# Atten4Vis/LW-DETR

Measured on AMD Instinct MI355X. Metric: images/sec, higher is better.
Workload: dtype fp16; 1 GPU; LW-DETR-small inference forward + PostProcess, 640x640, batch 32/GPU, fp16, random-init weights (synthetic COCO-shaped input); global_batch=32, per_gpu_batch=32, parallelism=dp1, collective=none, launch_chains=2

## Files before the change

lw-detr_amd/csrc/gemm.hip:

```cpp
#include "common.h"
#include <cstdlib>
#include <atomic>
#include <type_traits>

int lwdetr_gemm_pt_try(const lwdetr_gemm_desc& d, int dtype, hipStream_t st, bool& taken);

namespace {

constexpr int BK = 32;

template <typename T> __device__ __forceinline__ float act_apply(float x, int act) {
    if (act == ACT_GELU) return gelu_for<T>(x);
    if (act == ACT_SILU) return x * __builtin_amdgcn_rcpf(1.f + __expf(-x));
    if (act == ACT_RELU) return x > 0.f ? x : 0.f;
    return x;
}

__device__ __forceinline__ bool row_offset(const lwdetr_gemm_seg& sg, long m, long& off) {
    if (sg.mode == LWDETR_OUT_LINEAR) { off = m * sg.ldo; return true; }
    if (sg.mode == LWDETR_OUT_HEADS) {
        const int b = (int)(m / sg.p0), t = (int)(m - (long)b * sg.p0);
        off = ((long)b * sg.p2 * sg.p0 + t) * sg.p1;
        return true;
    }
// ... 750 lines not shown
    if constexpr (SPLITK) {
        constexpr int SLD = BN + 4, SLD_T = 64 + 4, SLAB = 64 * 68;
        float* stg = (float*)smem;
        int* flag = (int*)smem + SLAB + 16;
        static_assert((SLAB + 32) * 4 <= LDS_ELEMS * (int)sizeof(T), "stage + flag fit the ring area");
        {
            float* sp = col_orient ? stg + (wn * WN + l15) * SLD_T + wm * WM + g * 4 : stg + (wm * WM + l15) * SLD + wn * WN + g * 4;
            const int fs = col_orient ? 16 * SLD_T : 16, ts = col_orient ? 16 : 16 * SLD;
#pragma unroll
            for (int f = 0; f < FT; ++f)
#pragma unroll
                for (int t = 0; t < TT; ++t) *(f32x4*)(sp + f * fs + t * ts) = acc[f][t];
        }
        __syncthreads();
        float* ws = (float*)d.splitk_ws;
        const long ntiles = (long)gridDim.x / nsl;
        int* cnt = (int*)(ws + ntiles * nsl * SLAB);
        float* slab = ws + ((long)tile * nsl + slice) * SLAB;
        for (int i = tid; i < SLAB / 4; i += 256) ((f32x4*)slab)[i] = ((const f32x4*)stg)[i];
        asm volatile("s_waitcnt vmcnt(0)" ::: "memory");
        __syncthreads();
        if (tid == 0) {
            __builtin_amdgcn_fence(__ATOMIC_RELEASE, "agent");
            asm volatile("s_waitcnt vmcnt(0)" ::: "memory");
            *flag = __hip_atomic_fetch_add(cnt + tile, 1, __ATOMIC_RELAXED, __HIP_MEMORY_SCOPE_AGENT);
        }
        __syncthreads();
        if (*flag != nsl - 1) return;
        if (tid == 0) __builtin_amdgcn_fence(__ATOMIC_ACQUIRE, "agent");
        __syncthreads();
        const float* s0 = ws + (long)tile * nsl * SLAB;
        for (int i = tid; i < SLAB / 4; i += 256) {
            f32x4 a = ((const f32x4*)s0)[i];
            for (int s2 = 1; s2 < nsl; ++s2) { const f32x4 b = ((const f32x4*)(s0 + (long)s2 * SLAB))[i]; a[0] += b[0]; a[1] += b[1]; a[2] += b[2]; a[3] += b[3]; }
            ((f32x4*)stg)[i] = a;
        }
        if (tid == 0) __hip_atomic_store(cnt + tile, 0, __ATOMIC_RELAXED, __HIP_MEMORY_SCOPE_AGENT);
        __syncthreads();
        epilogue_finish<T, BN, 256>(d, sg, col_orient, stg, m0, n0);
    } else {
        gemm_epilogue<T, BM, BN>(d, sg, col_orient, acc, smem, m0, n0);
    }
}

template <typename T> struct Mma32;
template <> struct Mma32<f16> {
    static __device__ __forceinline__ f32x16 k16(f16x8 a, f16x8 b, f32x16 c) { return __builtin_amdgcn_mfma_f32_32x32x16_f16(a, b, c, 0, 0, 0); }
};
template <> struct Mma32<bf16> {
    static __device__ __forceinline__ f32x16 k16(bf16x8 a, bf16x8 b, f32x16 c) { return __builtin_amdgcn_mfma_f32_32x32x16_bf16(a, b, c, 0, 0, 0); }
};

#ifdef LWDETR_CONV_TIMING
__device__ unsigned long long g_conv_timing[4][12];
extern "C" int lwdetr_debug_conv_timing(unsigned long long* out) {
    return hipMemcpyFromSymbol(out, HIP_SYMBOL(g_conv_timing), sizeof(g_conv_timing)) == hipSuccess ? 0 : -1;
}
#define CONV_NOW() __builtin_amdgcn_s_memrealtime()
#endif
#ifndef LWDETR_CONV_ABL
#define LWDETR_CONV_ABL 0
#endif
template <typename V8>
__device__ __forceinline__ void lds_read16(V8& dst, unsigned lds_addr) { asm volatile("ds_read_b128 %0, %1" : "=v"(dst) : "v"(lds_addr)); }
__device__ __forceinline__ void divmod_magic(unsigned n, unsigned dvs, unsigned magic, unsigned& q, unsigned& r) {
    q = __umulhi(n, magic); r = n - q * dvs;
    if (r >= dvs) { ++q; r -= dvs; }
}

template <typename T, int CIN, int BN, int NST>
__global__ __launch_bounds__(256) void conv3x3_patch_kernel(const lwdetr_gemm_desc d, int np_patch, unsigned magic_hw, unsigned magic_w) {
    constexpr int BM = 128, KB = 32, EPC = 8;
    constexpr int SPR = CIN / EPC + 1, RS = SPR * EPC;
    constexpr int NCH = CIN / KB;
    constexpr int B_MY = BN / 16 / 4;
    constexpr int WN = BN / 2, TM = 2, TN = WN / 32, NRD = TM + TN;
    typedef typename Vec<T>::v8 V8;
    static_assert(sizeof(T) == 2 && BN % 64 == 0 && CIN % KB == 0 && (NCH == 4 || NCH == 6), "16-bit, whole pieces, 4 or 6 stages per tap");
    extern __shared__ __attribute__((aligned(16))) unsigned char conv_smem[];
    T* patch = (T*)conv_smem;
    T* ring = patch + (long)np_patch * 512;
    const unsigned lds_patch = (unsigned)(uintptr_t)(__attribute__((address_space(3))) void*)conv_smem;
    const unsigned lds_ring = lds_patch + (unsigned)np_patch * 1024u;

    const int nwg = gridDim.x;
    int wg;
    {
        const int bid = blockIdx.x, q = nwg >> 3, r = nwg & 7, xcd = bid & 7;
        wg = (xcd < r ? xcd * (q + 1) : r * (q + 1) + (xcd - r) * q) + (bid >> 3);
    }
    const int m0 = wg * BM;
    const int tid = threadIdx.x, lane = tid & 63, wave = tid >> 6;
    const int l31 = lane & 31, h = lane >> 5;
    const int wm = wave >> 1, wn = wave & 1;
    const int Wimg = d.conv_wout, Himg = d.conv_hout, PR = BM + 2 * Wimg + 2;
    const T* __restrict__ A = (const T*)d.A + d.a_col0;
    const T* __restrict__ W = (const T*)d.W;
    const T* zero = (const T*)g_zero16;
#ifdef LWDETR_CONV_TIMING
    const unsigned long long ct0 = CONV_NOW(); unsigned long long ct_lgkm = 0, ct_vm = 0, ct_bar = 0;
#endif

    const int prow = lane >> 2, pslot = lane & 3;
    const T* w_src[B_MY];
#pragma unroll
    for (int k = 0; k < B_MY; ++k) {
        const int n = 16 * (wave + 4 * k) + prow;
        w_src[k] = n < d.N ? W + (long)n * d.K + (pslot ^ ((prow >> 2) & 3)) * EPC : nullptr;
    }
    const int nk = 9 * NCH;
    auto stage = [&](int kt, int slot) {
        T* Bs = ring + slot * (BN * KB);
#pragma unroll
        for (int k = 0; k < B_MY; ++k) {
            if (LWDETR_CONV_ABL & 8) continue;
            gdma16((kt < nk && w_src[k]) ? w_src[k] + kt * KB : zero, Bs + (wave + 4 * k) * 64 * EPC);
        }
    };
#pragma unroll
    for (int s = 0; s < NST; ++s) stage(s, s);
    {
        constexpr unsigned MAGIC_SPR = 0x100000000ull / SPR;
        constexpr int DR = 256 / SPR, DS = 256 - DR * SPR;
        const int lda = (int)d.lda, gm0 = m0 - Wimg - 1;
        unsigned pr, ps;
        divmod_magic((unsigned)(wave * 64 + lane), SPR, MAGIC_SPR, pr, ps);
        int goff = (gm0 + (int)pr) * lda + (int)ps * EPC;
        for (int p = wave; p < np_patch; p += 4) {
            const int gm = gm0 + (int)pr;
            const bool ok = ps < SPR - 1 && (int)pr < PR && gm >= 0 && gm < d.M;
            if (!(LWDETR_CONV_ABL & 2)) gdma16(ok ? A + goff : zero, patch + p * 512);
            pr += DR; ps += DS; goff += DR * lda + DS * EPC;
            if (ps >= SPR) { ps -= SPR; ++pr; goff += lda - SPR * EPC; }
        }
    }
#ifdef LWDETR_CONV_TIMING
    const unsigned long long ct1 = CONV_NOW();
#endif
    unsigned vbits[TM], need[TM];
    {
        const unsigned hw = (unsigned)(Himg * Wimg);
#pragma unroll
        for (int i = 0; i < TM; ++i) {
            unsigned qq, r, y, x;
            divmod_magic((unsigned)(m0 + wm * 64 + i * 32 + l31), hw, magic_hw, qq, r);
            divmod_magic(r, (unsigned)Wimg, magic_w, y, x);
            const bool top = y == 0, bot = (int)y == Himg - 1, lef = x == 0, rig = (int)x == Wimg - 1;
            const unsigned row_ok[3] = {top ? 0u : 7u, 7u, bot ? 0u : 7u};
            const unsigned col_ok = (lef ? 0u : 0x49u) | 0x92u | (rig ? 0u : 0x124u);
            vbits[i] = (row_ok[0] | row_ok[1] << 3 | row_ok[2] << 6) & col_ok;
            const unsigned at = __builtin_amdgcn_ballot_w64(top) != 0, ab = __builtin_amdgcn_ballot_w64(bot) != 0;
            const unsigned al = __builtin_amdgcn_ballot_w64(lef) != 0, ar = __builtin_amdgcn_ballot_w64(rig) != 0;
            need[i] = (at ? 7u : 0u) | (ab ? 7u << 6 : 0u) | (al ? 0x49u : 0u) | (ar ? 0x124u : 0u);
        }
    }
    unsigned a_addr[TM], w_addr[TN][2];
#pragma unroll
    for (int i = 0; i < TM; ++i) a_addr[i] = lds_patch + (unsigned)(((wm * 64 + i * 32 + l31) * RS + h * EPC) * (int)sizeof(T));
#pragma unroll
    for (int j = 0; j < TN; ++j)
#pragma unroll
        for (int kc = 0; kc < 2; ++kc)
            w_addr[j][kc] = lds_ring + (unsigned)(((wn * WN + j * 32 + l31) * KB + ((2 * kc + h) ^ ((l31 >> 2) & 3)) * EPC) * (int)sizeof(T));

    f32x16 acc[TN][TM];
#pragma unroll
    for (int j = 0; j < TN; ++j)
#pragma unroll
        for (int i = 0; i < TM; ++i)
#pragma unroll
            for (int e = 0; e < 16; ++e) acc[j][i][e] = 0.f;

#ifdef LWDETR_CONV_TIMING
    const unsigned long long ct2 = CONV_NOW();
#endif
    wait_vmcnt<0>();
    __builtin_amdgcn_s_barrier();
#ifdef LWDETR_CONV_TIMING
    const unsigned long long ct3 = CONV_NOW();
#endif
    auto load = [&](auto c_tag, auto kc_tag, const unsigned (&a_tap)[TM], unsigned soff, V8 (&xf)[TM], V8 (&wf)[TN]) {
// ... 31 lines not shown
            for (int j = 0; j < TN; ++j) asm volatile("" :: "v"(wf[j]));
#pragma unroll
            for (int i = 0; i < TM; ++i) asm volatile("" :: "v"(xf[i]));
            return;
        }
#pragma unroll
        for (int j = 0; j < TN; ++j)
#pragma unroll
            for (int i = 0; i < TM; ++i) acc[j][i] = Mma32<T>::k16(wf[j], xf[i], acc[j][i]);
    };
    auto tap_rows = [&](int tap, unsigned (&a_tap)[TM]) {
        const unsigned toff = (unsigned)((Wimg + 1 + (tap / 3 - 1) * Wimg + (tap % 3 - 1)) * RS * (int)sizeof(T));
#pragma unroll
        for (int i = 0; i < TM; ++i) a_tap[i] = a_addr[i] + toff;
    };
    constexpr unsigned SLOT_B = BN * KB * sizeof(T);
    V8 xa[TM], wa[TN], xb[TM], wb[TN];
    unsigned a_cur[TM], a_nxt[TM];
    tap_rows(0, a_cur);
    load(std::integral_constant<int, 0>{}, std::integral_constant<int, 0>{}, a_cur, 0u, xa, wa);
    int kt = 0;
    unsigned soff = 0;
#pragma unroll 1
    for (int tap = 0; tap < 9; ++tap) {
        tap_rows(tap + 1, a_nxt);
        unsigned nd[TM], keep[TM];
#pragma unroll
        for (int i = 0; i < TM; ++i) { nd[i] = (need[i] >> tap) & 1; keep[i] = (vbits[i] >> tap) & 1 ? 0xffffffffu : 0u; }
        auto one_stage = [&](auto c_tag) {
            constexpr int C = decltype(c_tag)::value;
            load(c_tag, std::integral_constant<int, 1>{}, a_cur, soff, xb, wb);
            landed(std::integral_constant<int, NRD>{}, xa, wa);
            mma(nd, keep, xa, wa);
#ifdef LWDETR_CONV_TIMING
            const unsigned long long cta = CONV_NOW();
#endif
            landed(std::integral_constant<int, 0>{}, xb, wb);
#ifdef LWDETR_CONV_TIMING
            const unsigned long long ctb = CONV_NOW();
#endif
            wait_vmcnt<(NST - 2) * B_MY>();
#ifdef LWDETR_CONV_TIMING
            const unsigned long long ctc = CONV_NOW();
#endif
            __builtin_amdgcn_s_barrier();
#ifdef LWDETR_CONV_TIMING
            ct_lgkm += ctb - cta; ct_vm += ctc - ctb; ct_bar += CONV_NOW() - ctc;
#endif
            {
                T* Bs = (T*)((unsigned char*)ring + soff);
#pragma unroll
                for (int k = 0; k < B_MY; ++k) {
                    if (LWDETR_CONV_ABL & 8) continue;
                    gdma16((kt + NST < nk && w_src[k]) ? w_src[k] + (kt + NST) * KB : zero, Bs + (wave + 4 * k) * 64 * EPC);
                }
            }
            soff = soff + SLOT_B == NST * SLOT_B ? 0u : soff + SLOT_B;
            ++kt;
            if constexpr (C + 1 < NCH) load(std::integral_constant<int, C + 1>{}, std::integral_constant<int, 0>{}, a_cur, soff, xa, wa);
            else if (tap < 8) load(std::integral_constant<int, 0>{}, std::integral_constant<int, 0>{}, a_nxt, soff, xa, wa);
            mma(nd, keep, xb, wb);
        };
        one_stage(std::integral_constant<int, 0>{});
        one_stage(std::integral_constant<int, 1>{});
        one_stage(std::integral_constant<int, 2>{});
        one_stage(std::integral_constant<int, 3>{});
        if constexpr (NCH > 4) { one_stage(std::integral_constant<int, 4>{}); one_stage(std::integral_constant<int, 5>{}); }
#pragma unroll
        for (int i = 0; i < TM; ++i) a_cur[i] = a_nxt[i];
    }
#ifdef LWDETR_CONV_TIMING
    const unsigned long long ct4 = CONV_NOW();
#endif
    wait_vmcnt<0>();
    __syncthreads();
    float* stg = (float*)conv_smem;
    constexpr int SLD = BN + 4;
    if (LWDETR_CONV_ABL & 4) {
        float keepalive = 0.f;
#pragma unroll
        for (int j = 0; j < TN; ++j)
#pragma unroll
            for (int i = 0; i < TM; ++i)
#pragma unroll
                for (int e = 0; e < 16; ++e) keepalive += acc[j][i][e];
        if (keepalive == 123.456f) stg[0] = 1.f;
        return;
    }
#pragma unroll 1
    for (int pass = 0; pass < 2; ++pass) {
        if (wm == pass) {
#pragma unroll
            for (int i = 0; i < TM; ++i)
#pragma unroll
                for (int j = 0; j < TN; ++j)
#pragma unroll
                    for (int q = 0; q < 4; ++q) {
                        const f32x4 v = {acc[j][i][4 * q], acc[j][i][4 * q + 1], acc[j][i][4 * q + 2], acc[j][i][4 * q + 3]};
                        *(f32x4*)(stg + (i * 32 + l31) * SLD + wn * WN + j * 32 + q * 8 + h * 4) = v;
                    }
        }
        __syncthreads();
        epilogue_finish<T, BN, 256>(d, d.seg[0], false, stg, m0 + pass * 64, 0);
        __syncthreads();
    }
#ifdef LWDETR_CONV_TIMING
    if (wg == LWDETR_CONV_TIMING && lane == 0) {
        unsigned long long* o = g_conv_timing[wave];
        const unsigned long long ct5 = CONV_NOW();
        o[0] = ct1 - ct0; o[1] = ct2 - ct1; o[2] = ct3 - ct2; o[3] = ct4 - ct3; o[4] = ct5 - ct4; o[5] = ct_lgkm; o[6] = ct_vm; o[7] = ct_bar; o[8] = ct5 - ct0;
    }
#endif
}




#ifndef LWDETR_BIG_VARIANT
#define LWDETR_BIG_VARIANT 0
#endif
#ifdef LWDETR_BIG_TIMING
__device__ unsigned long long g_big_timing[8][8];
extern "C" int lwdetr_debug_big_timing(unsigned long long* out) {
    return hipMemcpyFromSymbol(out, HIP_SYMBOL(g_big_timing), sizeof(g_big_timing)) == hipSuccess ? 0 : 1;
}
#define BIG_NOW() __builtin_amdgcn_s_memrealtime()
#endif
template <typename T, int BN, int KB, int NST, int AMODE, int BM, int NW, bool LN = false>
__device__ __forceinline__ void gemm_big_body(const lwdetr_gemm_desc& d) {
    static_assert(sizeof(T) == 2, "16-bit types only");
    static_assert((NW == 8 && BM == 256) || (NW == 4 && BM == 128), "8 waves x 256 rows or 4 waves x 128 rows");
    constexpr int EPC = 8;
    constexpr int WGN = BN == 256 ? 4 : 2, WGM = NW / WGN;
    constexpr int WM = BM / WGM, WN = BN / WGN, TM = WM / 32, TN = WN / 32;
    static_assert(WN % 32 == 0 && WM % 64 == 0 && (BN / (64 / (KB / 8))) % NW == 0 && (BM / (64 / (KB / 8))) % NW == 0, "tile / stage combination not supported");
    constexpr int SLOTS = KB / EPC, RP = 64 / SLOTS, KC = KB / 16;
    constexpr int A_MY = BM / RP / NW, B_MY = BN / RP / NW, PER_STAGE = A_MY + B_MY;
    constexpr int STAGE = (BM + BN) * KB;
    typedef typename Vec<T>::v8 V8;
    extern __shared__ __attribute__((aligned(16))) char big_smem[];
    T* smem = (T*)big_smem;

    const int tiles_n = (d.N + BN - 1) / BN;
    int wg;
    {
        const int nwg = gridDim.x, bid = blockIdx.x, q = nwg >> 3, r = nwg & 7, xcd = bid & 7;
        wg = (xcd < r ? xcd * (q + 1) : r * (q + 1) + (xcd - r) * q) + (bid >> 3);
    }
    const int tm_ = wg / tiles_n, tn_ = wg - tm_ * tiles_n;
    const long m0 = (long)tm_ * BM;
    const int n0 = tn_ * BN;
    const int tid = threadIdx.x, lane = tid & 63, wave = tid >> 6;
    const int m = lane & 31, h = lane >> 5;
    const int wm = wave / WGN, wn = wave % WGN;
    const T* __restrict__ A = (const T*)d.A;
    const T* __restrict__ W = (const T*)d.W;
    const T* zero = (const T*)g_zero16;
// ... 240 lines not shown
}

int g_big_mode = -1;
template <int AMODE>
bool big_2wg_pays(const lwdetr_gemm_desc& d, int bn) {
    (void)d; (void)bn;
    return false;
}
template <typename T, int AMODE>
int try_launch_big(const lwdetr_gemm_desc& d, hipStream_t st, bool& taken) {
    taken = false;
    if constexpr (sizeof(T) != 2 || AMODE == LWDETR_A_PATCH16) return LWDETR_OK;
    else {
        const int mode = g_big_mode >= 0 ? g_big_mode : (int)lwdetr_knob(KNOB_GEMM_BIG, 1);
        if (!mode || d.A2 || d.K % 64 != 0 || d.N < 128) return LWDETR_OK;
        if (AMODE == LWDETR_A_CONV3x3 && (d.conv_cin % 64 != 0 || d.a_col0 % 8 != 0 || d.conv_hout > 1024 || d.conv_wout > 1024 ||
                                          d.M / ((long)d.conv_hout * d.conv_wout) >= 2048)) return LWDETR_OK;
        int bn = d.N % 256 == 0 || d.N > 512 ? 256 : (d.N <= 192 ? 192 : 128);
        bn = (int)lwdetr_knob(KNOB_GEMM_BIG_BN, bn);
        for (int s = 0; s < d.nseg; ++s)
            if (d.seg[s].n_begin % bn != 0) bn = 128;
        for (int s = 0; s < d.nseg; ++s) if (d.seg[s].n_begin % bn != 0) return LWDETR_OK;
        const long tiles = ((d.M + 255) / 256) * ((d.N + bn - 1) / bn);
        if (mode == 1 && !(d.K >= 384 && d.N >= 192 && (d.M >= 16384 || (d.K >= 960 && tiles >= 96)))) return LWDETR_OK;
        const int variant = mode >= 10 ? mode : 0;
        const int wg2_mode = (int)lwdetr_knob(KNOB_GEMM_BIG_2WG, 1);
        const bool wg2 = variant == 128 || (variant == 0 && (wg2_mode == 2 || (wg2_mode == 1 && big_2wg_pays<AMODE>(d, bn))));
        int rc;
        bool ln = false;
        for (int s_ = 0; s_ < d.nseg; ++s_) ln = ln || d.seg[s_].ln_stats != nullptr;
        if (ln) {
#ifdef LWDETR_EXPERIMENTS
            if constexpr (AMODE == LWDETR_A_PLAIN) {
                if (bn == 256) { rc = launch_big<T, 256, 64, 2, LWDETR_A_PLAIN, 256, 8, true>(d, st); taken = rc != LWDETR_ERR_UNSUPPORTED; return taken ? rc : LWDETR_OK; }
            }
#endif
            return LWDETR_OK;
        }
#ifdef LWDETR_EXPERIMENTS
        if (wg2 && bn == 256) rc = launch_big<T, 256, 32, 3, AMODE, 128, 4>(d, st);
        else if (wg2 && bn == 192) rc = launch_big<T, 192, 32, 3, AMODE, 128, 4>(d, st);
        else
#else
        (void)wg2;
#endif
        if (bn == 256) rc = variant == 32 ? launch_big<T, 256, 32, 4, AMODE>(d, st) : launch_big<T, 256, 64, 2, AMODE>(d, st);
        else if (bn == 192) rc = launch_big<T, 192, 64, 2, AMODE>(d, st);
        else rc = variant == 32 ? launch_big<T, 128, 32, 4, AMODE>(d, st) : launch_big<T, 128, 64, 3, AMODE>(d, st);
        taken = rc != LWDETR_ERR_UNSUPPORTED;
        return taken ? rc : LWDETR_OK;
    }
}

template <typename T, int CIN, int NST>
int launch_conv_patch(const lwdetr_gemm_desc& d, hipStream_t st) {
    constexpr int SPR = CIN / 8 + 1;
    const int pr = 128 + 2 * d.conv_wout + 2;
    const int np = (pr * SPR + 63) / 64;
    size_t lds = (size_t)np * 1024 + (size_t)NST * CIN * 32 * sizeof(T);
    const size_t stg = (size_t)64 * (CIN + 4) * sizeof(float);
    if (lds < stg) lds = stg;
    if (lds > 160 * 1024) return LWDETR_ERR_UNSUPPORTED;
    static signed char state[16] = {};
    int dev = 0;
    if (hipGetDevice(&dev) != hipSuccess || dev < 0 || dev >= 16) return LWDETR_ERR_UNSUPPORTED;
    if (state[dev] == 0)
        state[dev] = hipFuncSetAttribute((const void*)conv3x3_patch_kernel<T, CIN, CIN, NST>, hipFuncAttributeMaxDynamicSharedMemorySize, 160 * 1024) == hipSuccess ? 1 : -1;
    if (state[dev] < 0) { (void)hipGetLastError(); return LWDETR_ERR_UNSUPPORTED; }
    const long nwg = (d.M + 127) / 128;
    const unsigned hw = (unsigned)(d.conv_hout * d.conv_wout);
    hipLaunchKernelGGL((conv3x3_patch_kernel<T, CIN, CIN, NST>), dim3((unsigned)nwg), dim3(256), lds, st, d, np,
                       (unsigned)(0x100000000ull / hw), (unsigned)(0x100000000ull / (unsigned)d.conv_wout));
    return lwdetr_gemm_path_done(CIN == 128 ? GP_CONV_PATCH_128 : GP_CONV_PATCH_192, lwdetr_check_launch());
}

template <typename T>
int try_launch_conv_patch(const lwdetr_gemm_desc& d, hipStream_t st, bool& taken) {
    taken = false;
    if constexpr (sizeof(T) != 2) return LWDETR_OK;
    else {
        const int mode = (int)lwdetr_knob(KNOB_CONV_PATCH, 1);
        if (mode == 0) return LWDETR_OK;
        if (mode == 1 && d.N != 128) return LWDETR_OK;
        if (mode == 1 && d.M < 100 * 128) return LWDETR_OK;
        const lwdetr_gemm_seg& g = d.seg[0];
        const long hw = (long)d.conv_hout * d.conv_wout;
        if (d.conv_stride != 1 || d.a_tok.winmajor || d.a_tok.Hp != d.conv_hout || d.a_tok.Wp != d.conv_wout || d.nseg != 1 ||
            g.mode != LWDETR_OUT_LINEAR || d.N != d.conv_cin || d.K != 9 * d.conv_cin || (d.N != 128 && d.N != 192) ||
            d.lda % 8 != 0 || d.a_col0 % 8 != 0 || ((size_t)d.A & 15) != 0 || ((size_t)d.W & 15) != 0 || hw <= 1 || d.M % hw != 0 ||
            d.conv_wout < 2 || (long)(d.M + 256) * d.lda >= (1L << 30))
            return LWDETR_OK;
        const int rc = d.N == 128 ? launch_conv_patch<T, 128, 3>(d, st) : launch_conv_patch<T, 192, 3>(d, st);
        taken = rc != LWDETR_ERR_UNSUPPORTED;
        return taken ? rc : LWDETR_OK;
    }
}

template <typename T, int AMODE>
int launch(const lwdetr_gemm_desc& d, hipStream_t st) {
    bool bn64 = d.N <= 64 || sizeof(T) == 4;
    for (int s = 0; s < d.nseg; ++s)
        if ((d.seg[s].n_begin % 128) != 0) bn64 = true;
    const int BNsel = bn64 ? 64 : 128;
    for (int s = 0; s < d.nseg; ++s)
        if (d.seg[s].n_begin % BNsel != 0) return LWDETR_ERR_UNSUPPORTED;
    long tiles_m = (d.M + 127) / 128, tiles_n = (d.N + BNsel - 1) / BNsel;
    bool small = AMODE != LWDETR_A_CONV3x3 || tiles_m * tiles_n < 384;
    if (lwdetr_knob_is_set(KNOB_GEMM_TILE)) {
        const int tsel = (int)lwdetr_knob(KNOB_GEMM_TILE, 0);
        if (tsel == 1) small = true;
        if (tsel == 2) { small = false; bn64 = true; tiles_n = (d.N + 63) / 64; }
        if (tsel == 3 && !bn64) small = false;
    }
    if (small) { tiles_m = (d.M + 63) / 64; tiles_n = (d.N + 63) / 64; }
    const long nwg = tiles_m * tiles_n;
    if (nwg <= 0 || nwg > 0x7fffffffL) return LWDETR_ERR_BAD_ARG;
    const int kid = AMODE == LWDETR_A_PLAIN ? KID_GEMM : (AMODE == LWDETR_A_CONV3x3 ? KID_GEMM_CONV : KID_GEMM_PATCH);
    ProfScope ps(kid, 2.0 * d.M * d.N * d.K, ((double)d.M * d.K + (double)d.N * d.K + (double)d.M * d.N) * sizeof(T), st);
    if constexpr (AMODE == LWDETR_A_CONV3x3) {
        bool taken = false;
        const int rc = try_launch_conv_patch<T>(d, st, taken);
        if (taken) return rc;
    }
    if constexpr (AMODE == LWDETR_A_PLAIN && sizeof(T) == 2) {
        bool taken = false;
        const int rc = lwdetr_gemm_pt_try(d, std::is_same<T, f16>::value ? DT_F16 : DT_BF16, st, taken);
        if (taken) return rc;
    }
    {
        bool taken = false;
        const int rc = try_launch_big<T, AMODE>(d, st, taken);
        if (taken) return rc;
        for (int s_ = 0; s_ < d.nseg; ++s_)
            if (d.seg[s_].ln_stats) return LWDETR_ERR_UNSUPPORTED;
    }
    if constexpr (sizeof(T) == 2) {
        const int mode = (int)lwdetr_knob(KNOB_GEMM_DMA, 3);
        if (mode && !d.A2) {
            const bool kb64 = lwdetr_knob(KNOB_GEMM_KB, 32) == 64 && d.K % 64 == 0 && (AMODE != LWDETR_A_CONV3x3 || d.conv_cin % 64 == 0);
            int path;
            if (small && kb64) { hipLaunchKernelGGL((gemm_dma_kernel<T, 64, 64, AMODE, 3, 64>), dim3((unsigned)nwg), dim3(256), 0, st, d); path = GP_RING_64x64_D3_KB64; }
            else if (small) {
                const int nst = (int)lwdetr_knob(KNOB_GEMM_NST, 3);
                if (nst == 2) { hipLaunchKernelGGL((gemm_dma_kernel<T, 64, 64, AMODE, 2>), dim3((unsigned)nwg), dim3(256), 0, st, d); path = GP_RING_64x64_D2; }
#ifdef LWDETR_EXPERIMENTS
// ... 101 lines not shown
```

lw-detr_amd/csrc/topk.hip:

```cpp
#include "common.h"

namespace {

constexpr int TK_THREADS = 1024;
constexpr int TK_MAXK = 1024;
constexpr int TK_IDX_BITS = 20;
constexpr unsigned TK_IDX_MASK = (1u << TK_IDX_BITS) - 1;

__device__ __forceinline__ unsigned fkey(float f) {
    const unsigned u = __float_as_uint(f);
    return (u & 0x80000000u) ? ~u : (u | 0x80000000u);
}
__device__ __forceinline__ float fkey_inv(unsigned k) {
    return __uint_as_float((k & 0x80000000u) ? (k ^ 0x80000000u) : ~k);
}

__device__ __forceinline__ unsigned long long tk_comp(unsigned key, int i) {
    return ((unsigned long long)key << TK_IDX_BITS) | (unsigned long long)(TK_IDX_MASK - (unsigned)i);
}

struct TopkShared {
    unsigned hist[2048];
    unsigned long long sel[TK_MAXK];
    unsigned rank[TK_MAXK];
    unsigned bstar, above, cnt, nsel;
};

template <typename T, bool CACHE>
__device__ void topk_block(const T* __restrict__ x, int N, int K, TopkShared& sh, unsigned* __restrict__ keys) {
    const int tid = threadIdx.x;
    unsigned long long prefix = 0;
    unsigned rem = (unsigned)K;
    unsigned long long thr = 0;
    int top = 32 + TK_IDX_BITS;
    bool first = true;
    while (true) {
        const int bits = top > 30 ? 11 : 10;
        const int shift = top - bits;
        const unsigned nb = 1u << bits;
        for (int i = tid; i < 2048; i += TK_THREADS) sh.hist[i] = 0;
        __syncthreads();
        if (first) {
            int i = tid;
            for (; i + 3 * TK_THREADS < N; i += 4 * TK_THREADS) {
                unsigned k4[4];
#pragma unroll
                for (int u = 0; u < 4; ++u) k4[u] = fkey(to_f32<T>(x[i + u * TK_THREADS]));
#pragma unroll
                for (int u = 0; u < 4; ++u) {
                    if (CACHE) keys[i + u * TK_THREADS] = k4[u];
                    atomicAdd(&sh.hist[k4[u] >> 21], 1u);
                }
            }
            for (; i < N; i += TK_THREADS) {
                const unsigned k = fkey(to_f32<T>(x[i]));
                if (CACHE) keys[i] = k;
                atomicAdd(&sh.hist[k >> 21], 1u);
            }
        } else {
            for (int i = tid; i < N; i += TK_THREADS) {
                const unsigned long long c = tk_comp(CACHE ? keys[i] : fkey(to_f32<T>(x[i])), i);
                if ((c >> top) == prefix) atomicAdd(&sh.hist[(unsigned)(c >> shift) & (nb - 1)], 1u);
            }
        }
        first = false;
        __syncthreads();
        if (tid < 64) {
            const int per = (int)nb >> 6;
            unsigned own = 0;
            for (int j = 0; j < per; ++j) own += sh.hist[tid * per + ((j + tid) & (per - 1))];
            unsigned s = own;
#pragma unroll
            for (int o = 1; o < 64; o <<= 1) {
                const unsigned t = __shfl_down(s, o);
                if (tid + o < 64) s += t;
            }
            const unsigned excl = s - own;
            if (excl < rem && rem <= s) {
                unsigned acc = excl;
                for (int j = per - 1; j >= 0; --j) {
                    const unsigned c = sh.hist[tid * per + j];
                    if (acc + c >= rem) { sh.bstar = (unsigned)(tid * per + j); sh.above = acc; sh.cnt = c; break; }
                    acc += c;
                }
            }
        }
        __syncthreads();
        const unsigned bstar = sh.bstar, above = sh.above, cnt = sh.cnt;
        rem -= above;
        prefix = (prefix << bits) | bstar;
        top = shift;
        if (cnt == rem || top == 0) { thr = prefix << top; break; }
    }
    if (tid == 0) sh.nsel = 0;
    for (int i = tid; i < TK_MAXK; i += TK_THREADS) sh.rank[i] = 0;
    __syncthreads();
    for (int i = tid; i < N; i += TK_THREADS) {
        const unsigned long long c = tk_comp(CACHE ? keys[i] : fkey(to_f32<T>(x[i])), i);
        if (c >= thr) {
            const unsigned p = atomicAdd(&sh.nsel, 1u);
            if (p < (unsigned)K) sh.sel[p] = c;
        }
    }
    __syncthreads();
    const int parts = TK_THREADS / K > 0 ? TK_THREADS / K : 1;
    const int e = tid % K, p = tid / K;
    if (p < parts) {
        const unsigned long long mine = sh.sel[e];
        const int j0 = (int)((long)K * p / parts), j1 = (int)((long)K * (p + 1) / parts);
        unsigned r = 0;
        for (int j = j0; j < j1; ++j) r += sh.sel[j] > mine ? 1u : 0u;
        atomicAdd(&sh.rank[e], r);
    }
    __syncthreads();
}

template <typename T, bool CACHE>
__global__ __launch_bounds__(TK_THREADS) void topk_kernel(const T* __restrict__ x, int N, int K, int64_t* __restrict__ idx_out,
                                                          float* __restrict__ val_out) {
    __shared__ TopkShared sh;
    extern __shared__ unsigned tk_keys[];
    const int b = blockIdx.x;
    topk_block<T, CACHE>(x + (long)b * N, N, K, sh, tk_keys);
    const int tid = threadIdx.x;
    if (tid < K) {
        const unsigned long long c = sh.sel[tid];
        const unsigned r = sh.rank[tid];
        idx_out[(long)b * K + r] = (int64_t)(TK_IDX_MASK - (unsigned)(c & TK_IDX_MASK));
        if (val_out) val_out[(long)b * K + r] = fkey_inv((unsigned)(c >> TK_IDX_BITS));
    }
}

template <typename T, bool CACHE>
__global__ __launch_bounds__(TK_THREADS) void postprocess_kernel(const T* __restrict__ logits, const T* __restrict__ boxes,
                                                                 const float* __restrict__ sizes, int nq, int ncls, int K,
                                                                 float* __restrict__ scores, int64_t* __restrict__ labels,
                                                                 float* __restrict__ out_boxes, float* __restrict__ packed) {
    __shared__ TopkShared sh;
    extern __shared__ unsigned tk_keys[];
    const int b = blockIdx.x;
    const int N = nq * ncls;
    topk_block<T, CACHE>(logits + (long)b * N, N, K, sh, tk_keys);
    const int tid = threadIdx.x;
    if (tid < K) {
        const unsigned long long c = sh.sel[tid];
        const long o = (long)b * K + sh.rank[tid];
        const int i = (int)(TK_IDX_MASK - (unsigned)(c & TK_IDX_MASK));
        const int q = i / ncls;
        const float v = fkey_inv((unsigned)(c >> TK_IDX_BITS));
        const float score = to_f32<T>(from_f32<T>(1.f / (1.f + expf(-v))));
        const T* bx = boxes + ((long)b * nq + q) * 4;
        const float cx = to_f32<T>(bx[0]), cy = to_f32<T>(bx[1]);
        const float w = fmaxf(to_f32<T>(bx[2]), 0.f), h = fmaxf(to_f32<T>(bx[3]), 0.f);
        const float ih = sizes[b * 2], iw = sizes[b * 2 + 1];
        const float x0 = to_f32<T>(from_f32<T>(cx - 0.5f * w)) * iw, y0 = to_f32<T>(from_f32<T>(cy - 0.5f * h)) * ih;
        const float x1 = to_f32<T>(from_f32<T>(cx + 0.5f * w)) * iw, y1 = to_f32<T>(from_f32<T>(cy + 0.5f * h)) * ih;
        if (packed) {
            float* pr = packed + o * 6;
            pr[0] = score; pr[1] = (float)(i - q * ncls); pr[2] = x0; pr[3] = y0; pr[4] = x1; pr[5] = y1;
        } else {
            scores[o] = score;
            labels[o] = (int64_t)(i - q * ncls);
            out_boxes[o * 4 + 0] = x0; out_boxes[o * 4 + 1] = y0; out_boxes[o * 4 + 2] = x1; out_boxes[o * 4 + 3] = y1;
        }
    }
}

template <typename T>
__global__ __launch_bounds__(256) void rowmax_kernel(const T* __restrict__ x, long ld, long rows, int ncols, float* __restrict__ out) {
    constexpr int EPC = 4;
    typedef T VC __attribute__((ext_vector_type(EPC)));
    const int lane16 = threadIdx.x & 15;
    const long row = (long)blockIdx.x * 16 + (threadIdx.x >> 4);
    float m = -INFINITY;
    if (row < rows) {
        const T* xr = x + row * ld;
        const int full = ncols / EPC;
        for (int c = lane16; c < full; c += 16) {
            const VC t = *(const VC*)(xr + c * EPC);
#pragma unroll
            for (int e = 0; e < EPC; ++e) m = fmaxf(m, to_f32<T>(t[e]));
        }
        for (int c = full * EPC + lane16; c < ncols; c += 16) m = fmaxf(m, to_f32<T>(xr[c]));
    }
#pragma unroll
    for (int o = 8; o >= 1; o >>= 1) m = fmaxf(m, __shfl_xor(m, o));
    if (row < rows && lane16 == 0) out[row] = m;
}

}

constexpr size_t TK_CACHE_BYTES = 160 * 1024 - sizeof(TopkShared) - 256;
static bool tk_allow_lds(const void* fn) {
    static const void* done[16]; static int ndone = 0;
    for (int i = 0; i < ndone; ++i) if (done[i] == fn) return true;
    if (hipFuncSetAttribute(fn, hipFuncAttributeMaxDynamicSharedMemorySize, (int)TK_CACHE_BYTES) != hipSuccess) return false;
    if (ndone < 16) done[ndone++] = fn;
    return true;
}

#define LWDETR_DISPATCH_T(dtype, CALL)                 \
    switch (dtype) {                                   \
// ... 69 lines not shown
```

Baseline: 14100 images/sec.

## Add 8-wave 256-row conv3x3 patch kernel variant for large 128-channel convs

Templates the patch-based 3x3 conv kernel on wave count, adding an 8-wave variant with a 256-row M tile that loads the input patch and weight stages with more threads and does a single-pass epilogue. The wide variant (with 4 weight stages) is picked for 128-channel convs when the number of 128-row tiles exceeds the CU count. The aim is to amortise the halo patch load and weight streaming over more output rows and cut the tail wave. It raises LDS use per block, which may lower occupancy.

```diff
diff --git a/lw-detr_amd/csrc/gemm.hip b/lw-detr_amd/csrc/gemm.hip
--- a/lw-detr_amd/csrc/gemm.hip
+++ b/lw-detr_amd/csrc/gemm.hip
@@ -826,7 +826,7 @@
 };
 
 #ifdef LWDETR_CONV_TIMING
-__device__ unsigned long long g_conv_timing[4][12];
+__device__ unsigned long long g_conv_timing[8][12];
 extern "C" int lwdetr_debug_conv_timing(unsigned long long* out) {
     return hipMemcpyFromSymbol(out, HIP_SYMBOL(g_conv_timing), sizeof(g_conv_timing)) == hipSuccess ? 0 : -1;
 }
@@ -834,6 +834,9 @@
 #endif
 #ifndef LWDETR_CONV_ABL
 #define LWDETR_CONV_ABL 0
+#endif
+#ifndef LWDETR_CONV8_NST
+#define LWDETR_CONV8_NST 4
 #endif
 template <typename V8>
 __device__ __forceinline__ void lds_read16(V8& dst, unsigned lds_addr) { asm volatile("ds_read_b128 %0, %1" : "=v"(dst) : "v"(lds_addr)); }
@@ -842,15 +845,16 @@
     if (r >= dvs) { ++q; r -= dvs; }
 }
 
-template <typename T, int CIN, int BN, int NST>
-__global__ __launch_bounds__(256) void conv3x3_patch_kernel(const lwdetr_gemm_desc d, int np_patch, unsigned magic_hw, unsigned magic_w) {
-    constexpr int BM = 128, KB = 32, EPC = 8;
+template <typename T, int CIN, int BN, int NST, int NW>
+__global__ __launch_bounds__(NW * 64) void conv3x3_patch_kernel(const lwdetr_gemm_desc d, int np_patch, unsigned magic_hw, unsigned magic_w) {
+    constexpr int BM = NW * 32, KB = 32, EPC = 8;
     constexpr int SPR = CIN / EPC + 1, RS = SPR * EPC;
     constexpr int NCH = CIN / KB;
-    constexpr int B_MY = BN / 16 / 4;
+    constexpr int B_MY = BN / 16 / NW;
     constexpr int WN = BN / 2, TM = 2, TN = WN / 32, NRD = TM + TN;
     typedef typename Vec<T>::v8 V8;
-    static_assert(sizeof(T) == 2 && BN % 64 == 0 && CIN % KB == 0 && (NCH == 4 || NCH == 6), "16-bit, whole pieces, 4 or 6 stages per tap");
+    static_assert(sizeof(T) == 2 && BN % 64 == 0 && (BN / 16) % NW == 0 && CIN % KB == 0 && (NCH == 4 || NCH == 6) && (NW == 4 || NW == 8),
+                  "16-bit, whole pieces per wave, 4 or 6 stages per tap, 4 or 8 waves");
     extern __shared__ __attribute__((aligned(16))) unsigned char conv_smem[];
     T* patch = (T*)conv_smem;
     T* ring = patch + (long)np_patch * 512;
@@ -879,7 +883,7 @@
     const T* w_src[B_MY];
 #pragma unroll
     for (int k = 0; k < B_MY; ++k) {
-        const int n = 16 * (wave + 4 * k) + prow;
+        const int n = 16 * (wave + NW * k) + prow;
         w_src[k] = n < d.N ? W + (long)n * d.K + (pslot ^ ((prow >> 2) & 3)) * EPC : nullptr;
     }
     const int nk = 9 * NCH;
@@ -888,19 +892,19 @@
 #pragma unroll
         for (int k = 0; k < B_MY; ++k) {
             if (LWDETR_CONV_ABL & 8) continue;
-            gdma16((kt < nk && w_src[k]) ? w_src[k] + kt * KB : zero, Bs + (wave + 4 * k) * 64 * EPC);
+            gdma16((kt < nk && w_src[k]) ? w_src[k] + kt * KB : zero, Bs + (wave + NW * k) * 64 * EPC);
         }
     };
 #pragma unroll
     for (int s = 0; s < NST; ++s) stage(s, s);
     {
         constexpr unsigned MAGIC_SPR = 0x100000000ull / SPR;
-        constexpr int DR = 256 / SPR, DS = 256 - DR * SPR;
+        constexpr int DR = NW * 64 / SPR, DS = NW * 64 - DR * SPR;
         const int lda = (int)d.lda, gm0 = m0 - Wimg - 1;
         unsigned pr, ps;
         divmod_magic((unsigned)(wave * 64 + lane), SPR, MAGIC_SPR, pr, ps);
         int goff = (gm0 + (int)pr) * lda + (int)ps * EPC;
-        for (int p = wave; p < np_patch; p += 4) {
+        for (int p = wave; p < np_patch; p += NW) {
             const int gm = gm0 + (int)pr;
             const bool ok = ps < SPR - 1 && (int)pr < PR && gm >= 0 && gm < d.M;
             if (!(LWDETR_CONV_ABL & 2)) gdma16(ok ? A + goff : zero, patch + p * 512);
@@ -1038,7 +1042,7 @@
 #pragma unroll
                 for (int k = 0; k < B_MY; ++k) {
                     if (LWDETR_CONV_ABL & 8) continue;
-                    gdma16((kt + NST < nk && w_src[k]) ? w_src[k] + (kt + NST) * KB : zero, Bs + (wave + 4 * k) * 64 * EPC);
+                    gdma16((kt + NST < nk && w_src[k]) ? w_src[k] + (kt + NST) * KB : zero, Bs + (wave + NW * k) * 64 * EPC);
                 }
             }
             soff = soff + SLOT_B == NST * SLOT_B ? 0u : soff + SLOT_B;
@@ -1061,7 +1065,7 @@
     wait_vmcnt<0>();
     __syncthreads();
     float* stg = (float*)conv_smem;
-    constexpr int SLD = BN + 4;
+    constexpr int SLD = BN + 4, EPR = NW == 8 ? BM : 64;
     if (LWDETR_CONV_ABL & 4) {
         float keepalive = 0.f;
 #pragma unroll
@@ -1074,8 +1078,9 @@
         return;
     }
 #pragma unroll 1
-    for (int pass = 0; pass < 2; ++pass) {
-        if (wm == pass) {
+    for (int pass = 0; pass < BM / EPR; ++pass) {
+        if (wm * 64 / EPR == pass) {
+            const int r0 = wm * 64 - pass * EPR;
 #pragma unroll
             for (int i = 0; i < TM; ++i)
 #pragma unroll
@@ -1083,12 +1088,13 @@
 #pragma unroll
                     for (int q = 0; q < 4; ++q) {
                         const f32x4 v = {acc[j][i][4 * q], acc[j][i][4 * q + 1], acc[j][i][4 * q + 2], acc[j][i][4 * q + 3]};
-                        *(f32x4*)(stg + (i * 32 + l31) * SLD + wn * WN + j * 32 + q * 8 + h * 4) = v;
+                        *(f32x4*)(stg + (r0 + i * 32 + l31) * SLD + wn * WN + j * 32 + q * 8 + h * 4) = v;
                     }
         }
         __syncthreads();
-        epilogue_finish<T, BN, 256>(d, d.seg[0], false, stg, m0 + pass * 64, 0);
-        __syncthreads();
+#pragma unroll
+        for (int s = 0; s < EPR / 64; ++s) epilogue_finish<T, BN, NW * 64>(d, d.seg[0], false, stg + s * 64 * SLD, m0 + pass * EPR + s * 64, 0);
+        if (pass + 1 < BM / EPR) __syncthreads();
     }
 #ifdef LWDETR_CONV_TIMING
     if (wg == LWDETR_CONV_TIMING && lane == 0) {
@@ -1435,24 +1441,24 @@
     }
 }
 
-template <typename T, int CIN, int NST>
+template <typename T, int CIN, int NST, int NW>
 int launch_conv_patch(const lwdetr_gemm_desc& d, hipStream_t st) {
-    constexpr int SPR = CIN / 8 + 1;
-    const int pr = 128 + 2 * d.conv_wout + 2;
+    constexpr int SPR = CIN / 8 + 1, BM = NW * 32;
+    const int pr = BM + 2 * d.conv_wout + 2;
     const int np = (pr * SPR + 63) / 64;
     size_t lds = (size_t)np * 1024 + (size_t)NST * CIN * 32 * sizeof(T);
-    const size_t stg = (size_t)64 * (CIN + 4) * sizeof(float);
+    const size_t stg = (size_t)(NW == 8 ? BM : 64) * (CIN + 4) * sizeof(float);
     if (lds < stg) lds = stg;
     if (lds > 160 * 1024) return LWDETR_ERR_UNSUPPORTED;
     static signed char state[16] = {};
     int dev = 0;
     if (hipGetDevice(&dev) != hipSuccess || dev < 0 || dev >= 16) return LWDETR_ERR_UNSUPPORTED;
     if (state[dev] == 0)
-        state[dev] = hipFuncSetAttribute((const void*)conv3x3_patch_kernel<T, CIN, CIN, NST>, hipFuncAttributeMaxDynamicSharedMemorySize, 160 * 1024) == hipSuccess ? 1 : -1;
+        state[dev] = hipFuncSetAttribute((const void*)conv3x3_patch_kernel<T, CIN, CIN, NST, NW>, hipFuncAttributeMaxDynamicSharedMemorySize, 160 * 1024) == hipSuccess ? 1 : -1;
     if (state[dev] < 0) { (void)hipGetLastError(); return LWDETR_ERR_UNSUPPORTED; }
-    const long nwg = (d.M + 127) / 128;
+    const long nwg = (d.M + BM - 1) / BM;
     const unsigned hw = (unsigned)(d.conv_hout * d.conv_wout);
-    hipLaunchKernelGGL((conv3x3_patch_kernel<T, CIN, CIN, NST>), dim3((unsigned)nwg), dim3(256), lds, st, d, np,
+    hipLaunchKernelGGL((conv3x3_patch_kernel<T, CIN, CIN, NST, NW>), dim3((unsigned)nwg), dim3(NW * 64), lds, st, d, np,
                        (unsigned)(0x100000000ull / hw), (unsigned)(0x100000000ull / (unsigned)d.conv_wout));
     return lwdetr_gemm_path_done(CIN == 128 ? GP_CONV_PATCH_128 : GP_CONV_PATCH_192, lwdetr_check_launch());
 }
@@ -1471,9 +1477,20 @@
         if (d.conv_stride != 1 || d.a_tok.winmajor || d.a_tok.Hp != d.conv_hout || d.a_tok.Wp != d.conv_wout || d.nseg != 1 ||
             g.mode != LWDETR_OUT_LINEAR || d.N != d.conv_cin || d.K != 9 * d.conv_cin || (d.N != 128 && d.N != 192) ||
             d.lda % 8 != 0 || d.a_col0 % 8 != 0 || ((size_t)d.A & 15) != 0 || ((size_t)d.W & 15) != 0 || hw <= 1 || d.M % hw != 0 ||
-            d.conv_wout < 2 || (long)(d.M + 256) * d.lda >= (1L << 30))
+            d.conv_wout < 2 || (d.M + 512L + 2L * d.conv_wout) * d.lda >= (1L << 30))
             return LWDETR_OK;
-        const int rc = d.N == 128 ? launch_conv_patch<T, 128, 3>(d, st) : launch_conv_patch<T, 192, 3>(d, st);
+        static int ncu[16] = {};
+        int dev = 0;
+        if (hipGetDevice(&dev) != hipSuccess || dev < 0 || dev >= 16) return LWDETR_OK;
+        if (ncu[dev] == 0) {
+            int n = 0;
+            if (hipDeviceGetAttribute(&n, hipDeviceAttributeMultiprocessorCount, dev) != hipSuccess || n <= 0) n = 256;
+            ncu[dev] = n;
+        }
+        const bool wide = d.N == 128 && mode != 4 && (mode == 3 || (d.M + 127) / 128 > ncu[dev]);
+        int rc;
+        if (wide) rc = launch_conv_patch<T, 128, LWDETR_CONV8_NST, 8>(d, st);
+        else rc = d.N == 128 ? launch_conv_patch<T, 128, 3, 4>(d, st) : launch_conv_patch<T, 192, 3, 4>(d, st);
         taken = rc != LWDETR_ERR_UNSUPPORTED;
         return taken ? rc : LWDETR_OK;
     }
```

Result: no change. 14130 images/sec (median of 5 runs) (+0.2%).

## Rework radix-select top-k with native 16-bit keys, 12-bit digits and vector loads

Applied to the files above, without the earlier changes.

Radix selection in the top-k and postprocess kernels now uses the raw 16-bit half-precision bit pattern as the key instead of widening to float, so fewer radix passes are needed. Each pass uses 12-bit digits with a block-wide scan across all threads, and histogram clearing is folded into that scan. Inputs and cached keys are read with 4-wide vector loads. This cuts passes, global loads and synchronisations in the postprocess top-k, at the cost of extra shared memory and an alignment-dependent vector path.

```diff
diff --git a/lw-detr_amd/csrc/topk.hip b/lw-detr_amd/csrc/topk.hip
--- a/lw-detr_amd/csrc/topk.hip
+++ b/lw-detr_amd/csrc/topk.hip
@@ -6,6 +6,9 @@
 constexpr int TK_MAXK = 1024;
 constexpr int TK_IDX_BITS = 20;
 constexpr unsigned TK_IDX_MASK = (1u << TK_IDX_BITS) - 1;
+constexpr int TK_DIGIT = 12;
+constexpr int TK_BINS = 1 << TK_DIGIT;
+constexpr int TK_OWN = TK_BINS / TK_THREADS;
 
 __device__ __forceinline__ unsigned fkey(float f) {
     const unsigned u = __float_as_uint(f);
@@ -15,74 +18,113 @@
     return __uint_as_float((k & 0x80000000u) ? (k ^ 0x80000000u) : ~k);
 }
 
+template <typename T> struct TkKey {
+    static constexpr int BITS = 16;
+    static __device__ __forceinline__ unsigned of(T x) {
+        const unsigned u = __builtin_bit_cast(unsigned short, x);
+        return (u & 0x8000u) ? (~u & 0xFFFFu) : (u | 0x8000u);
+    }
+    static __device__ __forceinline__ float value(unsigned k) {
+        return to_f32<T>(__builtin_bit_cast(T, (unsigned short)((k & 0x8000u) ? (k ^ 0x8000u) : (~k & 0xFFFFu))));
+    }
+};
+template <> struct TkKey<float> {
+    static constexpr int BITS = 32;
+    static __device__ __forceinline__ unsigned of(float x) { return fkey(x); }
+    static __device__ __forceinline__ float value(unsigned k) { return fkey_inv(k); }
+};
+
 __device__ __forceinline__ unsigned long long tk_comp(unsigned key, int i) {
     return ((unsigned long long)key << TK_IDX_BITS) | (unsigned long long)(TK_IDX_MASK - (unsigned)i);
 }
 
 struct TopkShared {
-    unsigned hist[2048];
+    unsigned hist[TK_BINS];
     unsigned long long sel[TK_MAXK];
     unsigned rank[TK_MAXK];
+    unsigned wsum[TK_THREADS / 64];
     unsigned bstar, above, cnt, nsel;
 };
 
+template <typename T, bool FROM_LDS>
+__device__ __forceinline__ uint4 tk_load4(const T* __restrict__ x, const unsigned* __restrict__ keys, int g) {
+    if (FROM_LDS) return ((const uint4*)keys)[g];
+    const typename Vec<T>::v4 v = ((const typename Vec<T>::v4*)x)[g];
+    return make_uint4(TkKey<T>::of(v[0]), TkKey<T>::of(v[1]), TkKey<T>::of(v[2]), TkKey<T>::of(v[3]));
+}
+
 template <typename T, bool CACHE>
 __device__ void topk_block(const T* __restrict__ x, int N, int K, TopkShared& sh, unsigned* __restrict__ keys) {
-    const int tid = threadIdx.x;
+    typedef TkKey<T> KY;
+    const int tid = threadIdx.x, lane = tid & 63, wave = tid >> 6;
     unsigned long long prefix = 0;
     unsigned rem = (unsigned)K;
     unsigned long long thr = 0;
-    int top = 32 + TK_IDX_BITS;
+    int top = KY::BITS + TK_IDX_BITS;
     bool first = true;
+    const int NV = ((uintptr_t)x % (4 * sizeof(T))) == 0 && N >= 4 * TK_THREADS ? N >> 2 : 0;
+#pragma unroll
+    for (int j = 0; j < TK_OWN; ++j) sh.hist[tid * TK_OWN + j] = 0;
+    __syncthreads();
     while (true) {
-        const int bits = top > 30 ? 11 : 10;
+        const int bits = top < TK_DIGIT ? top : TK_DIGIT;
         const int shift = top - bits;
         const unsigned nb = 1u << bits;
-        for (int i = tid; i < 2048; i += TK_THREADS) sh.hist[i] = 0;
-        __syncthreads();
         if (first) {
-            int i = tid;
-            for (; i + 3 * TK_THREADS < N; i += 4 * TK_THREADS) {
-                unsigned k4[4];
-#pragma unroll
-                for (int u = 0; u < 4; ++u) k4[u] = fkey(to_f32<T>(x[i + u * TK_THREADS]));
+#pragma unroll 2
+            for (int g = tid; g < NV; g += TK_THREADS) {
+                const uint4 k4 = tk_load4<T, false>(x, keys, g);
+                if (CACHE) ((uint4*)keys)[g] = k4;
+                const unsigned kk[4] = {k4.x, k4.y, k4.z, k4.w};
+#pragma unroll
+                for (int u = 0; u < 4; ++u) atomicAdd(&sh.hist[kk[u] >> (KY::BITS - TK_DIGIT)], 1u);
+            }
+            for (int i = 4 * NV + tid; i < N; i += TK_THREADS) {
+                const unsigned k = KY::of(x[i]);
+                if (CACHE) keys[i] = k;
+                atomicAdd(&sh.hist[k >> (KY::BITS - TK_DIGIT)], 1u);
+            }
+        } else {
+#pragma unroll 2
+            for (int g = tid; g < NV; g += TK_THREADS) {
+                const uint4 k4 = tk_load4<T, CACHE>(x, keys, g);
+                const unsigned kk[4] = {k4.x, k4.y, k4.z, k4.w};
 #pragma unroll
                 for (int u = 0; u < 4; ++u) {
-                    if (CACHE) keys[i + u * TK_THREADS] = k4[u];
-                    atomicAdd(&sh.hist[k4[u] >> 21], 1u);
+                    const unsigned long long c = tk_comp(kk[u], 4 * g + u);
+                    if ((c >> top) == prefix) atomicAdd(&sh.hist[(unsigned)(c >> shift) & (nb - 1)], 1u);
                 }
             }
-            for (; i < N; i += TK_THREADS) {
-                const unsigned k = fkey(to_f32<T>(x[i]));
-                if (CACHE) keys[i] = k;
-                atomicAdd(&sh.hist[k >> 21], 1u);
-            }
-        } else {
-            for (int i = tid; i < N; i += TK_THREADS) {
-                const unsigned long long c = tk_comp(CACHE ? keys[i] : fkey(to_f32<T>(x[i])), i);
+            for (int i = 4 * NV + tid; i < N; i += TK_THREADS) {
+                const unsigned long long c = tk_comp(CACHE ? keys[i] : KY::of(x[i]), i);
                 if ((c >> top) == prefix) atomicAdd(&sh.hist[(unsigned)(c >> shift) & (nb - 1)], 1u);
             }
         }
         first = false;
         __syncthreads();
-        if (tid < 64) {
-            const int per = (int)nb >> 6;
-            unsigned own = 0;
-            for (int j = 0; j < per; ++j) own += sh.hist[tid * per + ((j + tid) & (per - 1))];
-            unsigned s = own;
-#pragma unroll
-            for (int o = 1; o < 64; o <<= 1) {
-                const unsigned t = __shfl_down(s, o);
-                if (tid + o < 64) s += t;
-            }
-            const unsigned excl = s - own;
-            if (excl < rem && rem <= s) {
-                unsigned acc = excl;
-                for (int j = per - 1; j >= 0; --j) {
-                    const unsigned c = sh.hist[tid * per + j];
-                    if (acc + c >= rem) { sh.bstar = (unsigned)(tid * per + j); sh.above = acc; sh.cnt = c; break; }
-                    acc += c;
-                }
+        unsigned c4[TK_OWN], own = 0;
+#pragma unroll
+        for (int j = 0; j < TK_OWN; ++j) {
+            const unsigned bin = (unsigned)(tid * TK_OWN + j);
+            c4[j] = bin < nb ? sh.hist[bin] : 0u;
+            sh.hist[bin] = 0;
+            own += c4[j];
+        }
+        unsigned s = own;
+#pragma unroll
+        for (int o = 1; o < 64; o <<= 1) {
+            const unsigned t = __shfl_down(s, o);
+            if (lane + o < 64) s += t;
+        }
+        if (lane == 0) sh.wsum[wave] = s;
+        __syncthreads();
+        for (int w = wave + 1; w < TK_THREADS / 64; ++w) s += sh.wsum[w];
+        unsigned acc = s - own;
+        if (acc < rem && rem <= s) {
+#pragma unroll
+            for (int j = TK_OWN - 1; j >= 0; --j) {
+                if (acc < rem && acc + c4[j] >= rem) { sh.bstar = (unsigned)(tid * TK_OWN + j); sh.above = acc; sh.cnt = c4[j]; }
+                acc += c4[j];
             }
         }
         __syncthreads();
@@ -95,8 +137,21 @@
     if (tid == 0) sh.nsel = 0;
     for (int i = tid; i < TK_MAXK; i += TK_THREADS) sh.rank[i] = 0;
     __syncthreads();
-    for (int i = tid; i < N; i += TK_THREADS) {
-        const unsigned long long c = tk_comp(CACHE ? keys[i] : fkey(to_f32<T>(x[i])), i);
+#pragma unroll 2
+    for (int g = tid; g < NV; g += TK_THREADS) {
+        const uint4 k4 = tk_load4<T, CACHE>(x, keys, g);
+        const unsigned kk[4] = {k4.x, k4.y, k4.z, k4.w};
+#pragma unroll
+        for (int u = 0; u < 4; ++u) {
+            const unsigned long long c = tk_comp(kk[u], 4 * g + u);
+            if (c >= thr) {
+                const unsigned p = atomicAdd(&sh.nsel, 1u);
+                if (p < (unsigned)K) sh.sel[p] = c;
+            }
+        }
+    }
+    for (int i = 4 * NV + tid; i < N; i += TK_THREADS) {
+        const unsigned long long c = tk_comp(CACHE ? keys[i] : KY::of(x[i]), i);
         if (c >= thr) {
             const unsigned p = atomicAdd(&sh.nsel, 1u);
             if (p < (unsigned)K) sh.sel[p] = c;
@@ -119,7 +174,7 @@
 __global__ __launch_bounds__(TK_THREADS) void topk_kernel(const T* __restrict__ x, int N, int K, int64_t* __restrict__ idx_out,
                                                           float* __restrict__ val_out) {
     __shared__ TopkShared sh;
-    extern __shared__ unsigned tk_keys[];
+    extern __shared__ __attribute__((aligned(16))) unsigned tk_keys[];
     const int b = blockIdx.x;
     topk_block<T, CACHE>(x + (long)b * N, N, K, sh, tk_keys);
     const int tid = threadIdx.x;
@@ -127,7 +182,7 @@
         const unsigned long long c = sh.sel[tid];
         const unsigned r = sh.rank[tid];
         idx_out[(long)b * K + r] = (int64_t)(TK_IDX_MASK - (unsigned)(c & TK_IDX_MASK));
-        if (val_out) val_out[(long)b * K + r] = fkey_inv((unsigned)(c >> TK_IDX_BITS));
+        if (val_out) val_out[(long)b * K + r] = TkKey<T>::value((unsigned)(c >> TK_IDX_BITS));
     }
 }
 
@@ -137,7 +192,7 @@
                                                                  float* __restrict__ scores, int64_t* __restrict__ labels,
                                                                  float* __restrict__ out_boxes, float* __restrict__ packed) {
     __shared__ TopkShared sh;
-    extern __shared__ unsigned tk_keys[];
+    extern __shared__ __attribute__((aligned(16))) unsigned tk_keys[];
     const int b = blockIdx.x;
     const int N = nq * ncls;
     topk_block<T, CACHE>(logits + (long)b * N, N, K, sh, tk_keys);
@@ -147,7 +202,7 @@
         const long o = (long)b * K + sh.rank[tid];
         const int i = (int)(TK_IDX_MASK - (unsigned)(c & TK_IDX_MASK));
         const int q = i / ncls;
-        const float v = fkey_inv((unsigned)(c >> TK_IDX_BITS));
+        const float v = TkKey<T>::value((unsigned)(c >> TK_IDX_BITS));
         const float score = to_f32<T>(from_f32<T>(1.f / (1.f + expf(-v))));
         const T* bx = boxes + ((long)b * nq + q) * 4;
         const float cx = to_f32<T>(bx[0]), cy = to_f32<T>(bx[1]);
```

Result: no change. 14770 images/sec before, 14840 images/sec after (median of 6 runs) (+0.5%).
